# FangjinhuaWang/PatchmatchNet

Measured on AMD Instinct MI355X. Metric: depth-maps/sec at 1600x1200 N=5 src views, higher is better.
Workload: dtype f32

## Files before the change

include/pmn_hip.h:

```cpp
#ifndef PMN_HIP_H
#define PMN_HIP_H

#include <stdint.h>

#ifdef __cplusplus
extern "C" {
#endif

#define PMN_ABI_VERSION 25
#define PMN_MLP_FLOATS 340
#define PMN_MAX_DEPTH 64
#define PMN_MAX_NEIGHBORS 17
#define PMN_MAX_FUSE_SRC 32
#define PMN_TSDF_MAX_VIEWS 16
#define PMN_TSDF_MARK_SPAN 8
#define PMN_RASTER_MAX_DIM 16384
#define PMN_RASTER_MAX_BOX 64
#define PMN_SPLAT_MAX_RADIUS 32

#define PMN_OK 0
#define PMN_ERR_ARG (-1)
#define PMN_ERR_SHAPE (-2)
#define PMN_ERR_LAUNCH (-3)

// ... 28 lines not shown
                          const float *feature_weight, const float *eval_offsets, const int *eval_table_host,
                          int K, float interval_scale, int is_inverse, int B, int D, int h, int w,
                          float *score_out, float *depth_out, void *stream);

int pmn_confidence(const float *score, int B, int D, int h, int w, int H, int W, float *confidence_out,
                   int *depth_index_out, void *stream);

int pmn_conv2d(const float *in, const float *weights, const float *shift, const float *up, float *out, int N, int H,
               int W, int cin, int cout, int K, int stride, int pad, int dil, int relu, int in_nchw, int out_nchw,
               int up_h, int up_w, void *stream);

int pmn_fpn_tail(const float *x, const float *up, const float *w_in, const float *b_in, const float *w_out, float *out,
                 int N, int H, int W, int cin, int cmid, int cout, void *stream);

int pmn_conv2d_mfma(const float *in, const float *weights, const float *shift, float *out, float *out_b, int N, int H, int W,
                    int cin, int cout, int ca, int K, int stride, int pad, int dil, int relu, int planar, void *stream);


int pmn_conv2d_f16s(const float *in, const void *weights, const float *shift, float *out, int N, int H, int W, int cin, int cout,
                    int k, int stride, int relu, void *stream);

int pmn_conv2d_f16s_pair(const float *in, const void *weights_a, const float *shift_a, const void *weights_b, const float *shift_b,
                         float *out, int N, int H, int W, int channels, int relu, void *stream);

int pmn_offset_heads_f16s(const float *in, const void *weights, const float *shift, float *out_a, float *out_b, int N, int H, int W,
                          int cin, int cout, int ca, int dil, void *stream);

int pmn_fpn_level(const float *x, const float *u, const float *w, const float *b, float *out_a, float *out_b, int N, int H,
                  int W, int cin, int cout, int ca, void *stream);

int pmn_deconv3x3s2(const float *in, const float *weights, const float *shift, float *out, int N, int Hi, int Wi, int cin,
                    int cout, int relu, void *stream);

int pmn_refine_front(const float *img, const float *t2, const float *w0, const float *s0, const float *wd, const float *sd,
                     float *x16, int B, int H, int W, void *stream);
int pmn_refine_tail(const float *x16, const float *w3, const float *s3, const float *wr, const float *dnorm,
                    const float *depth_min, const float *depth_max, float *out, int B, int H, int W, void *stream);

int pmn_refine_fused(const float *img, const float *t2, const float *w0, const float *s0, const float *wd, const float *sd,
                     const void *w3a, const float *s3, const float *wr, const float *dnorm, const float *depth_min,
                     const float *depth_max, float *out, int B, int H, int W, void *stream);

int pmn_stage_projections(const float *intrinsics, const float *extrinsics, int B, int V, int nstages, float scale0,
                          float *rel, void *stream);

int pmn_stem(const float *img, const float *w0, const float *s0, const float *w1, const float *s1, float *out, int N, int H,
             int W, void *stream);

int pmn_stem_f16s(const float *img, const float *w0, const float *s0, const void *w1a, const float *s1, float *out, int N, int H,
                  int W, void *stream);

int pmn_stem_f16s_views(const float *const *img_table, int views, const float *w0, const float *s0, const void *w1a,
                        const float *s1, float *out, int B, int H, int W, void *stream);

int pmn_differentiable_warping(const float *src_nchw, const float *rel_proj, const float *depth, int B, int C,
                               int D, int h, int w, int hs, int ws, float *warped, void *stream);

int pmn_fuse_view(const float *maps, long long slot_stride, int ref_slot, const int *src_slots_host,
                  const int *src_hw_host, int n_src, const float *mats, int H, int W, float geo_pixel_thres, float geo_depth_thres, int geo_mask_thres,
                  float photo_thres, unsigned char *masks, float *xyz, double *depth_avg, int *geo_sum, void *stream);

int pmn_fuse_view_merged(const float *maps, long long slot_stride, int ref_slot, const int *src_slots_host,
                         const int *src_hw_host, int n_src, const float *mats, int H, int W, float geo_pixel_thres,
                         float geo_depth_thres, int geo_mask_thres, float photo_thres, unsigned char *masks, float *xyz,
                         double *depth_avg, int *geo_sum, unsigned char *claimed, long long claim_stride, unsigned char *emit,
                         void *stream);

int pmn_pack_points(const unsigned char *final_mask, const float *xyz, const void *image_hwc, int image_is_float, int H, int W,
                    unsigned char *records, long long capacity_points, long long *cursor, int *view_count, long long *scratch,
                    void *stream);

int pmn_pack_points_normals(const unsigned char *final_mask, const float *xyz, const float *normals_chw, const float *rotation,
                            int rotation_stride, const void *image_hwc, int image_is_float, int H, int W, unsigned char *records,
                            long long capacity_points, long long *cursor, int *view_count, long long *scratch, void *stream);

int pmn_depth_normals(const float *depth, int H, int W, const float *intrinsics_host, int radius, float rel_thres,
                      float *normals_out, void *stream);

int pmn_normalize_depth(const float *depth, const float *depth_min, const float *depth_max, int B, int n, float *out,
                        void *stream);

int pmn_check_f16_domain(const float *x, long long n, int *flag, void *stream);

#define PMN_PLAN_PART_PRE 0
#define PMN_PLAN_PART_SIDE 1
#define PMN_PLAN_PART_MAIN 2
#define PMN_PLAN_PART_POST 3
int pmn_plan_create(void **plan_out);
int pmn_plan_begin(void *plan);
int pmn_plan_end(void *plan);
int pmn_plan_count(const void *plan);
const char *pmn_plan_kernel_name(const void *plan, int index);
int pmn_plan_launch(const void *plan, void *stream);
int pmn_plan_destroy(void *plan);
int pmn_plan_fork(void *plan);
int pmn_plan_switch(void *plan, int branch);
int pmn_plan_join(void *plan);
int pmn_plan_entry_branch(const void *plan, int index);
int pmn_plan_launch_part(const void *plan, int part, void *stream);

int pmn_view_scores(const double *cam_centers, const double *xyz, const long long *obs_ptr, const int *obs_pt,
                    const long long *trk_ptr, const int *trk_img, int N, int P, long long n_obs, long long n_trk,
                    double theta0, double sigma1, double sigma2, double *score, void *stream);

#define PMN_METRICS_MAX_STAGES 4
#define PMN_METRICS_MAX_ITERS 5
// ... 154 lines not shown
```

patchmatchnet_amd/_lib.py:

```python
from __future__ import annotations

import ctypes
import os
import subprocess
from typing import Optional

_CSRC = os.path.join(os.path.dirname(os.path.abspath(__file__)), "csrc")
LIB_PATH = os.path.join(_CSRC, "libpmn_hip.so")
ABI_VERSION = 25
MLP_FLOATS = 340
MAX_DEPTH = 64
MAX_NEIGHBORS = 17
MAX_FUSE_SRC = 32
TSDF_MAX_VIEWS = 16
TSDF_MARK_SPAN = 8
RASTER_MAX_DIM = 16384
RASTER_MAX_BOX = 64
SPLAT_MAX_RADIUS = 32
ICP_SUMS = 17
ICP_LIMBS = 5
ICP_BLOCK_POINTS = 256
VOXEL_LONG_RUN = 256
VOXEL_MAX_CHANNELS = 8
CROP_MAX_VERTICES = 4096
MESH_PLACE_LONG_RUN = 256
MESH_SIMPLIFY_MAX_FACES = 715827882
MESH_SMOOTH_LONG_ROW = 256
MESH_SMOOTH_MAX_STEPS = 65536
NORMAL_SWEEPS = 6
NORMAL_MAX_VIEWPOINTS = 4096
PLANE_MAX_HYPOTHESES = 4096
PLANE_SUMS = 10
PLANE_LIMBS = 5
PLANE_BLOCK_POINTS = 1024
MLS_QUADRIC_MIN = 6
MLS_PIVOT_MIN = 1e-10

_fp = ctypes.c_void_p
_ip = ctypes.c_void_p
_hp = ctypes.c_void_p
_i = ctypes.c_int
_f = ctypes.c_float
_s = ctypes.c_void_p

SIGNATURES = {
    "pmn_abi_version": [],
    "pmn_error_string": [_i],
    "pmn_nchw_to_nhwc": [_fp, _fp, _i, _i, _i, _i, _s],
    "pmn_feature_weight": [_fp, _fp, _hp, _fp, _i, _i, _i, _i, _i, _i, _fp, _s],
    "pmn_init_hypotheses": [_fp, _fp, _i, _fp, _fp, _i, _f, _fp, _hp, _i, _i, _i, _i, _fp, _fp, _s],
    "pmn_warp_correlate": [_fp, _fp, _fp, _fp, _fp, _i, _fp, _fp, _i, _i, _i, _i, _i, _i, _i, _i, _i, _fp, _fp, _ip,
                           _fp, _s],
    "pmn_warp_correlate_views": [_fp, _fp, _fp, _fp, _fp, _i, _fp, _fp, _i, _i, _i, _i, _i, _i, _i, _i, _i, _fp, _fp, _ip,
                                 _fp, _s],
    "pmn_aggregate_regress": [_fp, _fp, _fp, _fp, _fp, _hp, _i, _f, _i, _i, _i, _i, _i, _fp, _fp, _s],
    "pmn_confidence": [_fp, _i, _i, _i, _i, _i, _i, _fp, _ip, _s],
    "pmn_conv2d": [_fp, _fp, _fp, _fp, _fp] + [_i] * 14 + [_s],
    "pmn_fpn_tail": [_fp] * 6 + [_i] * 6 + [_s],
    "pmn_fpn_level": [_fp] * 6 + [_i] * 6 + [_s],
    "pmn_conv2d_f16s": [_fp] * 4 + [_i] * 8 + [_s],
    "pmn_offset_heads_f16s": [_fp] * 5 + [_i] * 7 + [_s],
    "pmn_conv2d_f16s_pair": [_fp] * 6 + [_i] * 5 + [_s],
    "pmn_refine_front": [_fp] * 7 + [_i] * 3 + [_s],
    "pmn_refine_tail": [_fp] * 8 + [_i] * 3 + [_s],
    "pmn_refine_fused": [_fp] * 13 + [_i] * 3 + [_s],
    "pmn_conv2d_mfma": [_fp] * 5 + [_i] * 12 + [_s],
    "pmn_deconv3x3s2": [_fp] * 4 + [_i] * 6 + [_s],
    "pmn_stage_projections": [_fp, _fp, _i, _i, _i, _f, _fp, _s],
    "pmn_stem": [_fp] * 6 + [_i] * 3 + [_s],
    "pmn_stem_f16s": [_fp] * 6 + [_i] * 3 + [_s],
    "pmn_stem_f16s_views": [_fp, _i] + [_fp] * 5 + [_i] * 3 + [_s],
    "pmn_differentiable_warping": [_fp, _fp, _fp, _i, _i, _i, _i, _i, _i, _i, _fp, _s],
    "pmn_fuse_view": [_fp, ctypes.c_longlong, _i, _hp, _hp, _i, _fp, _i, _i, _f, _f, _i, _f, _fp, _fp, _fp, _ip, _s],
    "pmn_fuse_view_merged": [_fp, ctypes.c_longlong, _i, _hp, _hp, _i, _fp, _i, _i, _f, _f, _i, _f, _fp, _fp, _fp, _ip, _fp,
                             ctypes.c_longlong, _fp, _s],
    "pmn_pack_points": [_fp, _fp, _fp, _i, _i, _i, _fp, ctypes.c_longlong, _fp, _ip, _fp, _s],
    "pmn_pack_points_normals": [_fp, _fp, _fp, _fp, _i, _fp, _i, _i, _i, _fp, ctypes.c_longlong, _fp, _ip, _fp, _s],
    "pmn_depth_normals": [_fp, _i, _i, _hp, _i, _f, _fp, _s],
    "pmn_normalize_depth": [_fp, _fp, _fp, _i, _i, _fp, _s],
    "pmn_check_f16_domain": [_fp, ctypes.c_longlong, _ip, _s],
    "pmn_plan_create": [ctypes.POINTER(ctypes.c_void_p)],
    "pmn_plan_begin": [_hp],
    "pmn_plan_end": [_hp],
    "pmn_plan_count": [_hp],
    "pmn_plan_kernel_name": [_hp, _i],
    "pmn_plan_launch": [_hp, _s],
    "pmn_plan_destroy": [_hp],
    "pmn_plan_fork": [_hp],
    "pmn_plan_switch": [_hp, _i],
    "pmn_plan_join": [_hp],
    "pmn_plan_entry_branch": [_hp, _i],
    "pmn_plan_launch_part": [_hp, _i, _s],
    "pmn_view_scores": [_fp] * 6 + [_i, _i, ctypes.c_longlong, ctypes.c_longlong] + [ctypes.c_double] * 3 + [_fp, _s],
    "pmn_depth_metrics": [_fp, _fp, _hp, _hp, _hp, _i, _hp, _i, _i, _i, _i, _fp, ctypes.c_longlong, _fp, _s],
    "pmn_nn_distance": [_fp, _ip, ctypes.c_longlong, _hp, ctypes.c_double, _hp, _fp, _ip, ctypes.c_longlong, ctypes.c_double, _fp, _ip,
                        _s],
    "pmn_reduce_round": [_fp, _ip, ctypes.c_longlong, _hp, ctypes.c_double, _hp, ctypes.c_double, _ip, _ip, _ip, _s],
    "pmn_tsdf_integrate": [_fp] * 4 + [_hp, _hp, _f, _f, _fp, ctypes.c_longlong] + [_hp] * 5 + [_i, _s],
    "pmn_mt_count": [_fp, _fp, _hp, _f, _ip, _ip, _s],
    "pmn_mt_emit": [_fp] * 4 + [_hp, _hp, _f, _f] + [_ip] * 4 + [_fp, _ip, _fp, _ip, _s],
    "pmn_tsdf_mark_blocks": [_ip, _ip, _hp, _hp, _f, _f, _fp, ctypes.c_longlong] + [_hp] * 4 + [_i, _s],
    "pmn_tsdf_integrate_blocks": [_fp] * 4 + [_ip, _i, _hp, _hp, _f, _f, _fp, ctypes.c_longlong] + [_hp] * 5 + [_i, _s],
    "pmn_mt_count_blocks": [_fp, _fp, _ip, _ip, _i, _hp, _f, _ip, _ip, _s],
    "pmn_mt_emit_blocks": [_fp] * 4 + [_ip, _ip, _i, _hp, _hp, _f, _f] + [_ip] * 4 + [_fp, _ip, _fp, _ip, _s],
    "pmn_raster_triangles": [_fp, _i, _ip, _i, _hp, _i, _i, ctypes.c_longlong, _ip, _ip, _ip, _s],
    "pmn_splat_points": [_fp, ctypes.c_longlong, _hp, _i, _i, _f, _f, _ip, _ip, _s],
    "pmn_raster_resolve": [_ip, _i, _i, _hp, _fp, ctypes.c_longlong, _ip, ctypes.c_longlong, _ip, _fp, _i, _fp, _ip, _ip, _fp, _s],
    "pmn_icp_accumulate": [_fp, _ip, ctypes.c_longlong, _hp, ctypes.c_double, _hp, _fp, _ip, ctypes.c_longlong, _hp, _hp, ctypes.c_double,
                           _fp, ctypes.c_longlong, _fp, _s],
    "pmn_voxel_mean": [_fp, _fp, _i, ctypes.c_longlong, _ip, ctypes.c_longlong, _fp, _fp, _s],
    "pmn_crop_prism": [_fp, ctypes.c_longlong, _fp, _i, _i, ctypes.c_double, ctypes.c_double, _hp, _ip, _s],
    "pmn_mesh_components": [_ip, _i, _i, _ip, _ip, _s],
    "pmn_mesh_face_samples": [_fp, _i, _ip, _i, ctypes.c_double, ctypes.c_ulonglong, _ip, _ip, _s],
    "pmn_mesh_sample": [_fp, _i, _ip, _i, _ip, _ip, ctypes.c_longlong, ctypes.c_ulonglong, _fp, _ip, _ip, _s],
    "pmn_undistort_image": [_fp, _i, _i, _i, _i, _hp, _hp, _i, _i, _fp, _fp, _fp, _s],
    "pmn_knn_distance": [_fp, _ip, ctypes.c_longlong, _hp, ctypes.c_double, _hp, _fp, _ip, ctypes.c_longlong, _i, ctypes.c_double, _i,
                         _fp, _ip, _fp, _s],
    "pmn_radius_count": [_fp, _ip, ctypes.c_longlong, _hp, ctypes.c_double, _hp, _fp, _ip, ctypes.c_longlong, ctypes.c_double, _i, _ip,
                         _s],
    "pmn_knn_normals": [_fp, _ip, ctypes.c_longlong, _hp, ctypes.c_double, _hp, _fp, _ip, ctypes.c_longlong, _i, ctypes.c_double, _i,
                        _fp, _i, ctypes.c_double, _fp, _fp, _ip, _s],
    "pmn_cloud_core": [_fp, _ip, ctypes.c_longlong, _hp, ctypes.c_double, _hp, ctypes.c_double, ctypes.c_longlong, _ip, _s],
    "pmn_cloud_dbscan": [_fp, _ip, ctypes.c_longlong, _hp, ctypes.c_double, _hp, ctypes.c_double, _ip, _ip, _ip, _ip, _s],
    "pmn_plane_score": [_fp, _fp, _ip, ctypes.c_longlong, _fp, _i, ctypes.c_double, ctypes.c_double, _ip, _s],
# ... 87 lines not shown
```

patchmatchnet_amd/csrc/conv_f16s.hip:

```cpp
#include "conv_common.hpp"

struct F16sArgs {
    int N, H, W, Ho, Wo, relu;
    int cout, ca;
    float* out_b;
};

template <int CIN, int COUT, int KS, int S, int CC, int CCP, int MT, int WPS, int DIL = 1, int OUTMODE = 0, bool SWAP = (OUTMODE == 0)>
__global__ __launch_bounds__(256, WPS) void conv_f16s_kernel(const float* __restrict__ in, const f16x8* __restrict__ wB,
                                                             const float* __restrict__ shift, float* __restrict__ out,
                                                             const F16sArgs a) {
    constexpr int NT = COUT / 16, NCB = CC / 8, CHUNKS = CIN / CC, NQ = KS * KS * NCB, KSTEPS = (NQ + 3) / 4;
    constexpr int TH = 4 * MT, TW = 16, PH = (TH - 1) * S + (KS - 1) * DIL + 1, PW = (TW - 1) * S + (KS - 1) * DIL + 1;
    constexpr int PAD = DIL * (KS / 2);
    constexpr int PLANE = PH * PW * CCP;
    constexpr int NTHR = 256;
    static_assert(!SWAP || OUTMODE == 0, "swapped operand roles (see the epilogue) serve the channels-last output");
    static_assert(CCP % 8 == 0 && CC % 8 == 0 && CIN % CC == 0, "16-byte aligned channel blocks");
    extern __shared__ float4 f16s_lds4[];
    _Float16* Phi = reinterpret_cast<_Float16*>(f16s_lds4);
    _Float16* Plo = Phi + PLANE;
    const int tid = threadIdx.x, wave = __builtin_amdgcn_readfirstlane(tid >> 6), lane = tid & 63, li = lane & 15, kb = lane >> 4;
    const int tiles_x = (a.Wo + TW - 1) / TW, tiles_y = (a.Ho + TH - 1) / TH;
    const int bt = pmn_xcd_tile(blockIdx.x, a.N * tiles_x * tiles_y);
// ... 491 lines not shown
        q = q < 8 ? q : 8;
        const int dy = q / 3, dx = q - dy * 3;
        const _Float16* pb = midh + ((wrow + dy) * MRP + li + dx) * 8;
        f16x8 bh[4], blo[4];
#pragma unroll
        for (int t = 0; t < 4; ++t) {
            bh[t] = *reinterpret_cast<const f16x8*>(pb + t * MRP * 8);
            blo[t] = *reinterpret_cast<const f16x8*>(pb + t * MRP * 8 + MROWS * MRP * 8);
        }
#pragma unroll
        for (int t = 0; t < 4; ++t) accM[t] = __builtin_amdgcn_mfma_f32_16x16x32_f16(wa[ks][0], bh[t], accM[t], 0, 0, 0);
#pragma unroll
        for (int t = 0; t < 4; ++t) accL[t] = __builtin_amdgcn_mfma_f32_16x16x32_f16(wa[ks][0], blo[t], accL[t], 0, 0, 0);
#pragma unroll
        for (int t = 0; t < 4; ++t) accL[t] = __builtin_amdgcn_mfma_f32_16x16x32_f16(wa[ks][1], bh[t], accL[t], 0, 0, 0);
    }
    const int ox = ox0 + li, oyw = oy0 + wrow;
    if (kb < 2 && ox < W) {
        const f32x4_t sh = *reinterpret_cast<const f32x4_t*>(s1 + 4 * kb);
        float* po = out + (((size_t)n * H + oyw) * W + ox) * 8 + 4 * kb;
        const size_t rs = (size_t)W * 8;
#pragma unroll
        for (int t = 0; t < 4; ++t) {
            if (oyw + t < H) {
                *reinterpret_cast<f32x4_t*>(po + t * rs) = f16s_relu(f16s_epilogue(accM[t], accL[t], sh));
            }
        }
    }
    }
}

static int launch_stem_f16s(const float* img, const float* const* img_table, int B, bool vec4, const float* w0, const float* s0,
                            const void* w1a, const float* s1, float* out, int N, int H, int W, void* stream) {
    constexpr int TS = 16, TH = PMN_STEM_TH;
    const int blocks = N * ((W + TS - 1) / TS) * ((H + TH - 1) / TH);
    PMN_LAUNCH((vec4 ? stem_f16s_kernel<true, PMN_STEM_TH> : stem_f16s_kernel<false, PMN_STEM_TH>), dim3(blocks), dim3(256), 0,
               (hipStream_t)stream, img, w0, s0, reinterpret_cast<const f16x8*>(w1a), s1, out, N, H, W, img_table, B);
    PMN_CHECK_LAUNCH();
    return PMN_OK;
}

extern "C" int pmn_stem_f16s(const float* img, const float* w0, const float* s0, const void* w1a, const float* s1, float* out,
                             int N, int H, int W, void* stream) {
    if (!img || !w0 || !s0 || !w1a || !s1 || !out || N < 1 || H < 1 || W < 1) return PMN_ERR_ARG;
    const bool vec4 = W % 4 == 0 && (reinterpret_cast<uintptr_t>(img) & 15) == 0;
    return launch_stem_f16s(img, nullptr, 1, vec4, w0, s0, w1a, s1, out, N, H, W, stream);
}

extern "C" int pmn_stem_f16s_views(const float* const* img_table, int views, const float* w0, const float* s0, const void* w1a,
                                   const float* s1, float* out, int B, int H, int W, void* stream) {
    if (!img_table || !w0 || !s0 || !w1a || !s1 || !out || views < 1 || B < 1 || H < 1 || W < 1) return PMN_ERR_ARG;
    return launch_stem_f16s(nullptr, img_table, B, W % 4 == 0, w0, s0, w1a, s1, out, views * B, H, W, stream);
}
```

patchmatchnet_amd/net.py:

```python
from __future__ import annotations

from typing import Dict, List, Optional, Tuple

import warnings

import numpy as np
import torch
import torch.nn as nn
import torch.nn.functional as F

from . import _lib, ops, params
from ._lib import PmnError
from .module import ConvBnReLU
from .patchmatch import PatchMatch


class FeatureNet(nn.Module):

    def __init__(self) -> None:
        super().__init__()
        spec = [(3, 8, 3, 1, 1), (8, 8, 3, 1, 1), (8, 16, 5, 2, 2), (16, 16, 3, 1, 1), (16, 16, 3, 1, 1),
                (16, 32, 5, 2, 2), (32, 32, 3, 1, 1), (32, 32, 3, 1, 1), (32, 64, 5, 2, 2), (64, 64, 3, 1, 1),
                (64, 64, 3, 1, 1)]
        for i, (cin, cout, k, s, p) in enumerate(spec):
            setattr(self, f"conv{i}", ConvBnReLU(cin, cout, k, s, p))
        self.output1 = nn.Conv2d(64, 64, 1, bias=False)
        self.inner1 = nn.Conv2d(32, 64, 1, bias=True)
        self.inner2 = nn.Conv2d(16, 64, 1, bias=True)
        self.output2 = nn.Conv2d(64, 32, 1, bias=False)
        self.output3 = nn.Conv2d(64, 16, 1, bias=False)
        self.f16_split = True
        self.f16_domain_error: Optional[str] = None
        self.fold_fpn = True
        self.fuse_conv34 = True
        self.fpn8_valu = False
        self.layer_hook = None

    _SPEC = [(3, 1, 1), (3, 1, 1), (5, 2, 2), (3, 1, 1), (3, 1, 1), (5, 2, 2), (3, 1, 1), (3, 1, 1), (5, 2, 2), (3, 1, 1),
             (3, 1, 1)]

    def _packed(self):
        srcs = [p for p in self.parameters()] + [b for b in self.buffers() if b.dtype.is_floating_point]
        key = params.versions(srcs)
        if getattr(self, "_pack_key", None) != key:
            dev = self.output1.weight.device
            pk = {}
            f16_ok, self.f16_domain_error = True, None
            for i in range(11):
                m = getattr(self, f"conv{i}")
                w, s = params.pack_conv(m.conv.weight, bn=(m.bn.weight, m.bn.bias, m.bn.running_mean, m.bn.running_var),
                                        eps=m.bn.eps)
                pk[f"conv{i}"] = (torch.from_numpy(w).to(dev), torch.from_numpy(s).to(dev))
                cv = m.conv
                if (cv.kernel_size[0], cv.stride[0], cv.in_channels, cv.out_channels) in ops.F16S_SHAPES and f16_ok:
                    try:
                        w, s = params.pack_conv_f16s(cv.weight, bn=(m.bn.weight, m.bn.bias, m.bn.running_mean, m.bn.running_var),
                                                     eps=m.bn.eps)
                        pk[f"conv{i}_f16s"] = (torch.from_numpy(w).to(dev), torch.from_numpy(s).to(dev))
                    except params.F16DomainError as e:
                        f16_ok, self.f16_domain_error = False, f"conv{i}: {e}"
            m1 = self.conv1
            try:
                w, s = params.pack_stem_conv1_f16s(m1.conv.weight, bn=(m1.bn.weight, m1.bn.bias, m1.bn.running_mean, m1.bn.running_var),
                                                  eps=m1.bn.eps)
                pk["conv1_f16s"] = (torch.from_numpy(w).to(dev), torch.from_numpy(s).to(dev))
            except params.F16DomainError as e:
                f16_ok, self.f16_domain_error = False, f"conv1: {e}"
            if not f16_ok:
                for k in [k for k in pk if k.endswith("_f16s")]:
                    del pk[k]
                warnings.warn("FeatureNet: " + self.f16_domain_error + " -- using the fp32 kernels (pmn_stem / pmn_conv2d) instead of "
                              "the fp16-split matrix-core kernels", RuntimeWarning, stacklevel=2)
            for name in ("output1", "inner1", "inner2", "output2", "output3"):
                m = getattr(self, name)
                w, s = params.pack_conv(m.weight, bias=m.bias)
                pk[name] = (torch.from_numpy(w).to(dev), torch.from_numpy(s).to(dev))
            fold = params.fold_fpn(self.output1.weight, self.inner1.weight, self.inner1.bias, self.inner2.weight,
                                   self.inner2.bias, self.output2.weight, self.output3.weight)
            for lvl, (w, b) in fold.items():
                pk[f"fpn{lvl}"] = (torch.from_numpy(w).to(dev), torch.from_numpy(b).to(dev))
            w8 = torch.from_numpy(np.ascontiguousarray(fold[8][0].T))[:, :, None, None]
            w, s = params.pack_conv_mfma(w8, bias=torch.from_numpy(fold[8][1]))
            pk["fpn8_mfma"] = (torch.from_numpy(w).to(dev), torch.from_numpy(s).to(dev))
            self._pack, self._pack_key = pk, key
        return self._pack

    def forward_hip(self, x, image_table: Optional["ops.SourceTable"] = None, pending: Optional[dict] = None
                    ) -> Dict[int, torch.Tensor]:
        pk = self._packed()
        imgs = list(x) if isinstance(x, (list, tuple)) else [x]
        B, _, H, W = imgs[0].shape
        in_place = image_table is not None
        if in_place and not (self.f16_split and "conv1_f16s" in pk):
            raise PmnError("image_table: only the fp16-split stem (FeatureNet.f16_split, weights inside its domain) reads images in place")
        if in_place:
            t = ops.stem_f16s_views(image_table, *pk["conv0"], *pk["conv1_f16s"])
        else:
            t = torch.empty((B * len(imgs), H, W, 8), dtype=torch.float32, device=imgs[0].device)
        for i, im in enumerate(() if in_place else imgs):
            if self.f16_split and "conv1_f16s" in pk:
                ops.stem_f16s(im.contiguous(), *pk["conv0"], *pk["conv1_f16s"], out=t[i * B:(i + 1) * B])
            else:
                ops.stem(im.contiguous(), *pk["conv0"], *pk["conv1"], out=t[i * B:(i + 1) * B])
        feats = {}
        for i, (k, s, p) in enumerate(self._SPEC):
            if i < 2:
                continue
            if i == 4 and self.f16_split and self.fuse_conv34 and "conv3_f16s" in pk and "conv4_f16s" in pk:
                continue
            if i == 3 and self.f16_split and self.fuse_conv34 and "conv3_f16s" in pk and "conv4_f16s" in pk:
                t = ops.conv2d_f16s_pair(t, *pk["conv3_f16s"], *pk["conv4_f16s"], relu=True)
                feats[4] = t
            elif self.f16_split and f"conv{i}_f16s" in pk:
                t = ops.conv2d_f16s(t, *pk[f"conv{i}_f16s"], k, s, relu=True)
            elif self.layer_hook is not None and (hooked := self.layer_hook(i, t)) is not None:
                t = hooked
            else:
                w, sh = pk[f"conv{i}"]
                t = ops.conv2d(t, w, sh, getattr(self, f"conv{i}").conv.out_channels, k, s, p, relu=True)
            if i in (4, 7, 10):
                feats[i] = t
        half, quarter, eighth = feats[4], feats[7], feats[10]
        if self.fold_fpn:
            if self.fpn8_valu:
                f3, u8 = ops.fpn_level(eighth, None, *pk["fpn8"], ca=64)
            else:
                f3, u8 = ops.pointwise_split_mfma(eighth, *pk["fpn8_mfma"], cout=112, ca=64)
            if pending is not None:
                pending.update(half=half, quarter=quarter, u8=u8)
                return {3: f3}
            return {3: f3, **self.finish_hip(dict(half=half, quarter=quarter, u8=u8))}
        out = {3: ops.conv2d(eighth, *pk["output1"], 64, 1)}
        top = ops.conv2d(quarter, *pk["inner1"], 64, 1, up=eighth)
        out[2] = ops.conv2d(top, *pk["output2"], 32, 1)
        out[1] = ops.fpn_tail(half, top, pk["inner2"][0], pk["inner2"][1], pk["output3"][0])
        return out

    def finish_hip(self, pending: dict) -> Dict[int, torch.Tensor]:
        pk = self._packed()
        f2, u4 = ops.fpn_level(pending["quarter"], pending["u8"], *pk["fpn4"], ca=32)
        f1, _ = ops.fpn_level(pending["half"], u4, *pk["fpn2"], ca=16)
        return {2: f2, 1: f1}

    def forward(self, x: torch.Tensor) -> Dict[int, torch.Tensor]:
        half = self.conv4(self.conv3(self.conv2(self.conv1(self.conv0(x)))))
        quarter = self.conv7(self.conv6(self.conv5(half)))
        eighth = self.conv10(self.conv9(self.conv8(quarter)))
        out: Dict[int, torch.Tensor] = {3: self.output1(eighth)}
        top = F.interpolate(eighth, scale_factor=2.0, mode="bilinear", align_corners=False) + self.inner1(quarter)
        out[2] = self.output2(top)
        top = F.interpolate(top, scale_factor=2.0, mode="bilinear", align_corners=False) + self.inner2(half)
        out[1] = self.output3(top)
        return out


class Refinement(nn.Module):

    def __init__(self) -> None:
        super().__init__()
# ... 268 lines not shown
```

patchmatchnet_amd/ops.py:

```python
from __future__ import annotations

import ctypes
import threading
from typing import List, Optional, Sequence, Tuple

import numpy as np
import torch

from . import _lib
from ._lib import PmnError, check


_TIMING = None
_TIMING_ON = True


def enable_kernel_timing() -> None:
    global _TIMING, _TIMING_ON
    _TIMING, _TIMING_ON = [], True


def pause_kernel_timing(paused: bool) -> None:
    global _TIMING_ON
    _TIMING_ON = not paused
# ... 759 lines not shown
def stem(img: torch.Tensor, w0: torch.Tensor, s0: torch.Tensor, w1: torch.Tensor, s1: torch.Tensor,
         out: Optional[torch.Tensor] = None) -> torch.Tensor:
    for n_, t_ in (("img", img), ("w0", w0), ("s0", s0), ("w1", w1), ("s1", s1)):
        _dev(t_, n_)
    N, c, H, W = img.shape
    if c != 3 or tuple(w0.shape) != (3, 3, 3, 8) or tuple(w1.shape) != (3, 3, 8, 8):
        raise PmnError("stem: expects a 3-channel image and 3->8->8 weights")
    if out is None:
        out = torch.empty((N, H, W, 8), dtype=torch.float32, device=img.device)
    else:
        _dev(out, "out")
        if tuple(out.shape) != (N, H, W, 8):
            raise PmnError("stem: bad `out` shape")
    with torch.cuda.device(img.device):
        check(_lib.lib().pmn_stem(img.data_ptr(), w0.data_ptr(), s0.data_ptr(), w1.data_ptr(), s1.data_ptr(), out.data_ptr(),
                                  N, H, W, _stream(img)), "pmn_stem")
    return out


def stem_f16s(img: torch.Tensor, w0: torch.Tensor, s0: torch.Tensor, w1a: torch.Tensor, s1: torch.Tensor,
              out: Optional[torch.Tensor] = None) -> torch.Tensor:
    for n_, t_ in (("img", img), ("w0", w0), ("s0", s0), ("s1", s1)):
        _dev(t_, n_)
    if tuple(_dev_as(w1a, "stem_f16s: w1a", torch.float16).shape) != (3, 2, 64, 8):
        raise PmnError("stem_f16s: w1a must be the float16 [3,2,64,8] tensor of params.pack_stem_conv1_f16s")
    N, c, H, W = img.shape
    if c != 3 or tuple(w0.shape) != (3, 3, 3, 8):
        raise PmnError("stem_f16s: expects a 3-channel image and 3->8 conv0 weights")
    _f16_domain_probe(img)
    if out is None:
        out = torch.empty((N, H, W, 8), dtype=torch.float32, device=img.device)
    else:
        _dev(out, "out")
        if tuple(out.shape) != (N, H, W, 8):
            raise PmnError("stem_f16s: bad `out` shape")
    with torch.cuda.device(img.device):
        check(_lib.lib().pmn_stem_f16s(img.data_ptr(), w0.data_ptr(), s0.data_ptr(), w1a.data_ptr(), s1.data_ptr(), out.data_ptr(),
                                       N, H, W, _stream(img)), "pmn_stem_f16s")
    return out


def stem_f16s_views(images: "SourceTable", w0: torch.Tensor, s0: torch.Tensor, w1a: torch.Tensor, s1: torch.Tensor) -> torch.Tensor:
    for n_, t_ in (("w0", w0), ("s0", s0), ("s1", s1)):
        _dev(t_, n_)
    if not isinstance(images, SourceTable) or len(images.shape) != 5 or images.shape[2] != 3:
        raise PmnError("stem_f16s_views: a SourceTable of shape (views, B, 3, H, W)")
    if tuple(_dev_as(w1a, "stem_f16s_views: w1a", torch.float16).shape) != (3, 2, 64, 8) or tuple(w0.shape) != (3, 3, 3, 8):
        raise PmnError("stem_f16s_views: 3->8 conv0 weights and the float16 [3,2,64,8] tensor of params.pack_stem_conv1_f16s")
    V, B, _, H, W = images.shape
    out = torch.empty((V * B, H, W, 8), dtype=torch.float32, device=images.device)
    with torch.cuda.device(images.device):
        check(_lib.lib().pmn_stem_f16s_views(images.table.data_ptr(), V, w0.data_ptr(), s0.data_ptr(), w1a.data_ptr(), s1.data_ptr(),
                                             out.data_ptr(), B, H, W, _stream(out)), "pmn_stem_f16s_views")
    return out


def fuse_view(maps: torch.Tensor, ref_slot: int, src_slots: Sequence[int], mats: torch.Tensor, geo_pixel_thres: float,
              geo_depth_thres: float, geo_mask_thres: int, photo_thres: float, want_depth_avg: bool = False,
              want_geo_sum: bool = False, sizes: Optional[Sequence[Tuple[int, int]]] = None):
    masks, xyz, davg, gsum, _ = _fuse_view(maps, ref_slot, src_slots, mats, geo_pixel_thres, geo_depth_thres, geo_mask_thres,
                                           photo_thres, want_depth_avg, want_geo_sum, sizes, None)
    return masks, xyz, davg, gsum


def fuse_view_merged(maps: torch.Tensor, ref_slot: int, src_slots: Sequence[int], mats: torch.Tensor, geo_pixel_thres: float,
                     geo_depth_thres: float, geo_mask_thres: int, photo_thres: float, claimed: torch.Tensor,
                     sizes: Optional[Sequence[Tuple[int, int]]] = None):
    if not isinstance(claimed, torch.Tensor) or claimed.dtype != torch.uint8 or claimed.dim() != 2 or not claimed.is_contiguous():
        raise PmnError("fuse_view_merged: claimed must be a contiguous uint8 tensor [V,S], one slot per map slot")
    if not isinstance(maps, torch.Tensor) or claimed.device != maps.device:
        raise PmnError("fuse_view_merged: claimed must be on the maps' device (no CPU fallback)")
    if ref_slot in src_slots:
        raise PmnError("fuse_view_merged: the reference slot is in its own source list")
    masks, xyz, _, _, emit = _fuse_view(maps, ref_slot, src_slots, mats, geo_pixel_thres, geo_depth_thres, geo_mask_thres,
                                        photo_thres, False, False, sizes, claimed)
    return masks, xyz, emit


def _fuse_view(maps, ref_slot, src_slots, mats, geo_pixel_thres, geo_depth_thres, geo_mask_thres, photo_thres, want_depth_avg,
               want_geo_sum, sizes, claimed):
    _dev(maps, "maps")
    _dev(mats, "mats")
    if sizes is None:
        if maps.dim() != 4 or maps.shape[1] != 2:
            raise PmnError("fuse_view: maps must be [V,2,H,W] (or [V,F] flat slots with sizes=)")
        V, _, H, W = maps.shape
        stride = 2 * H * W
        sizes = [(H, W)] * V
    else:
        if maps.dim() != 2 or len(sizes) != maps.shape[0]:
            raise PmnError("fuse_view: with sizes= maps must be [V,F] flat slots and sizes must have V entries")
        V, stride = maps.shape
        if any(h < 1 or w < 1 or 2 * h * w > stride for h, w in sizes):
            raise PmnError("fuse_view: a view's maps do not fit its slot")
    n = len(src_slots)
    if n > _lib.MAX_FUSE_SRC:
        raise PmnError(f"fuse_view: at most {_lib.MAX_FUSE_SRC} source views per reference view")
    if not 0 <= ref_slot < V or any(not 0 <= s < V for s in src_slots):
        raise PmnError("fuse_view: slot out of range")
    if mats.numel() != 48 + 64 * n:
        raise PmnError("fuse_view: mats must hold 48 + 64 * n_src floats (fusion.camera_block)")
    if claimed is not None and (claimed.shape[0] != V or any(h * w > claimed.shape[1] for h, w in sizes)):
        raise PmnError("fuse_view_merged: claimed must have one slot per map slot, each with room for the largest view's h*w bytes")
    H, W = sizes[ref_slot]
    slots, slots_p = _host_i32(np.asarray(list(src_slots) if n else [0], np.int32), max(n, 1), "src_slots")
    hw, hw_p = _host_i32(np.asarray([x for s in src_slots for x in sizes[s]] if n else [0, 0], np.int32), max(2 * n, 2), "src_hw")
# ... 630 lines not shown
```

Measured before the change: 400.9.

## Fuse stem conv0/conv1 with stride-2 conv2 in one LDS-resident kernel

Adds a kernel that computes conv0 and conv1 of the feature stem into LDS as fp16 hi/lo split planes, then runs the 5x5 stride-2 conv2 from LDS with MFMA. It writes only the half-resolution 16-channel output. This removes the full-resolution 8-channel intermediate write and read, plus a launch. In exchange it recomputes halo regions per 16x16 output tile and uses large LDS per block, which limits occupancy.

```diff
diff --git a/include/pmn_hip.h b/include/pmn_hip.h
--- a/include/pmn_hip.h
+++ b/include/pmn_hip.h
@@ -104,6 +104,12 @@
 
 int pmn_stem_f16s_views(const float *const *img_table, int views, const float *w0, const float *s0, const void *w1a,
                         const float *s1, float *out, int B, int H, int W, void *stream);
+
+int pmn_stem_conv2_f16s(const float *img, const float *w0, const float *s0, const void *w1a, const float *s1, const void *w2b,
+                        const float *s2, float *out, int N, int H, int W, void *stream);
+
+int pmn_stem_conv2_f16s_views(const float *const *img_table, int views, const float *w0, const float *s0, const void *w1a,
+                              const float *s1, const void *w2b, const float *s2, float *out, int B, int H, int W, void *stream);
 
 int pmn_differentiable_warping(const float *src_nchw, const float *rel_proj, const float *depth, int B, int C,
                                int D, int h, int w, int hs, int ws, float *warped, void *stream);
diff --git a/patchmatchnet_amd/_lib.py b/patchmatchnet_amd/_lib.py
--- a/patchmatchnet_amd/_lib.py
+++ b/patchmatchnet_amd/_lib.py
@@ -70,6 +70,8 @@
     "pmn_stem": [_fp] * 6 + [_i] * 3 + [_s],
     "pmn_stem_f16s": [_fp] * 6 + [_i] * 3 + [_s],
     "pmn_stem_f16s_views": [_fp, _i] + [_fp] * 5 + [_i] * 3 + [_s],
+    "pmn_stem_conv2_f16s": [_fp] * 8 + [_i] * 3 + [_s],
+    "pmn_stem_conv2_f16s_views": [_fp, _i] + [_fp] * 7 + [_i] * 3 + [_s],
     "pmn_differentiable_warping": [_fp, _fp, _fp, _i, _i, _i, _i, _i, _i, _i, _fp, _s],
     "pmn_fuse_view": [_fp, ctypes.c_longlong, _i, _hp, _hp, _i, _fp, _i, _i, _f, _f, _i, _f, _fp, _fp, _fp, _ip, _s],
     "pmn_fuse_view_merged": [_fp, ctypes.c_longlong, _i, _hp, _hp, _i, _fp, _i, _i, _f, _f, _i, _f, _fp, _fp, _fp, _ip, _fp,
diff --git a/patchmatchnet_amd/csrc/conv_f16s.hip b/patchmatchnet_amd/csrc/conv_f16s.hip
--- a/patchmatchnet_amd/csrc/conv_f16s.hip
+++ b/patchmatchnet_amd/csrc/conv_f16s.hip
@@ -567,3 +567,252 @@
     if (!img_table || !w0 || !s0 || !w1a || !s1 || !out || views < 1 || B < 1 || H < 1 || W < 1) return PMN_ERR_ARG;
     return launch_stem_f16s(nullptr, img_table, B, W % 4 == 0, w0, s0, w1a, s1, out, views * B, H, W, stream);
 }
+
+
+template <int J>
+__device__ __forceinline__ void stem_conv2_conv1_tiles(const _Float16* __restrict__ m0h, _Float16* __restrict__ m1h, const f16x8 (&wa)[3][2],
+                                                       const f32x4_t sh1, const int first, const int ntiles, const int lim, const int g0,
+                                                       const int wave, const int li, const int kb, const int yc, const int xc, const int H,
+                                                       const int W) {
+    constexpr int C0 = 37, C1 = 35, M0PLANE = 37 * 37 * 8, M1PLANE = 35 * 35 * 8;
+    f32x4_t accM[J], accL[J];
+    const _Float16* pb[J];
+    int mm[J];
+#pragma unroll
+    for (int j = 0; j < J; ++j) {
+        accM[j] = f32x4_t{0.f, 0.f, 0.f, 0.f};
+        accL[j] = f32x4_t{0.f, 0.f, 0.f, 0.f};
+        const int t = wave + 8 * (g0 + j);
+        const int m = min(first + (t < ntiles ? t : ntiles - 1) * 16 + li, lim - 1);
+        mm[j] = t < ntiles && first + t * 16 + li < lim ? m : -1;
+        const int r = m / C1, c = m - r * C1;
+        pb[j] = m0h + (r * C0 + c) * 8;
+    }
+#pragma unroll
+    for (int ks = 0; ks < 3; ++ks) {
+        int q = 4 * ks + kb;
+        q = q < 8 ? q : 8;
+        const int dy = q / 3, dx = q - dy * 3;
+        const int off = (dy * C0 + dx) * 8;
+        f16x8 bh[J], blo[J];
+#pragma unroll
+        for (int j = 0; j < J; ++j) {
+            bh[j] = *reinterpret_cast<const f16x8*>(pb[j] + off);
+            blo[j] = *reinterpret_cast<const f16x8*>(pb[j] + off + M0PLANE);
+        }
+#pragma unroll
+        for (int j = 0; j < J; ++j) accM[j] = __builtin_amdgcn_mfma_f32_16x16x32_f16(wa[ks][0], bh[j], accM[j], 0, 0, 0);
+#pragma unroll
+        for (int j = 0; j < J; ++j) accL[j] = __builtin_amdgcn_mfma_f32_16x16x32_f16(wa[ks][0], blo[j], accL[j], 0, 0, 0);
+#pragma unroll
+        for (int j = 0; j < J; ++j) accL[j] = __builtin_amdgcn_mfma_f32_16x16x32_f16(wa[ks][1], bh[j], accL[j], 0, 0, 0);
+    }
+    if (kb < 2) {
+#pragma unroll
+        for (int j = 0; j < J; ++j) {
+            const int m = mm[j];
+            if (m >= 0) {
+                const int r = m / C1, c = m - r * C1;
+                f16x4 hi = {0, 0, 0, 0}, lo = {0, 0, 0, 0};
+                if ((unsigned)(yc + r) < (unsigned)H && (unsigned)(xc + c) < (unsigned)W)
+                    f16s_split4(f16s_relu(f16s_epilogue(accM[j], accL[j], sh1)), hi, lo);
+                *reinterpret_cast<f16x4*>(m1h + m * 8 + 4 * kb) = hi;
+                *reinterpret_cast<f16x4*>(m1h + M1PLANE + m * 8 + 4 * kb) = lo;
+            }
+        }
+    }
+}
+
+template <bool VEC4>
+__global__ __launch_bounds__(512, 4) void stem_f16s_kernel_conv2(const float* __restrict__ img, const float* __restrict__ w0,
+                                                                const float* __restrict__ s0, const f16x8* __restrict__ w1A,
+                                                                const float* __restrict__ s1, const f16x8* __restrict__ w2B,
+                                                                const float* __restrict__ s2, float* __restrict__ out, const int N,
+                                                                const int H, const int W, const int Ho, const int Wo,
+                                                                const float* const* __restrict__ img_tab, const int BV) {
+    constexpr int TO = 16, NTHR = 512;
+    constexpr int IR = 39, IC = 40;
+    constexpr int R0 = 37, C0 = 37;
+    constexpr int R1 = 35, C1 = 35;
+    constexpr int M0PLANE = R0 * C0 * 8, M1PLANE = R1 * C1 * 8;
+    constexpr int LATE = 3 * C1;
+    static_assert((R1 * C1 - LATE) % 16 == 0, "the early part of conv1 is whole tiles");
+    extern __shared__ float4 sc2_lds4[];
+    _Float16* m0h = reinterpret_cast<_Float16*>(sc2_lds4);
+    _Float16* m1h = m0h + 2 * M0PLANE - LATE * 8;
+    float* xin = reinterpret_cast<float*>(m0h + 2 * M0PLANE);
+    typedef const float __attribute__((address_space(4))) cfloat;
+    const cfloat* cw0 = (const cfloat*)w0;
+    const cfloat* cs0 = (const cfloat*)s0;
+    const int tid = threadIdx.x, wave = __builtin_amdgcn_readfirstlane(tid >> 6), lane = tid & 63, li = lane & 15, kb = lane >> 4;
+    const int tiles_x = (Wo + TO - 1) / TO, tiles_y = (Ho + TO - 1) / TO;
+    const int bt = pmn_xcd_tile(blockIdx.x, N * tiles_x * tiles_y);
+    const int n = bt / (tiles_x * tiles_y), tr = bt - n * tiles_x * tiles_y;
+    const int oy0 = (tr / tiles_x) * TO, ox0 = (tr % tiles_x) * TO;
+    const int yi = 2 * oy0 - 4, xi = 2 * ox0 - 4;
+    if (img_tab) img = img_tab[n / BV] + (ptrdiff_t)((n % BV) - n) * 3 * H * W;
+
+    f16x8 wa[3][2];
+#pragma unroll
+    for (int ks = 0; ks < 3; ++ks) {
+        wa[ks][0] = w1A[(ks * 2 + 0) * 64 + lane];
+        wa[ks][1] = w1A[(ks * 2 + 1) * 64 + lane];
+    }
+    if constexpr (VEC4) {
+        constexpr int NU = (3 * IR + 31) / 32;
+        float4 v[NU];
+        const int j = tid & 15, gx = xi + 4 * j;
+#pragma unroll
+        for (int u = 0; u < NU; ++u) {
+            const int R = (tid >> 4) + 32 * u;
+            const int c = (R >= IR) + (R >= 2 * IR), r = R - IR * c, gy = yi + r;
+            v[u] = make_float4(0.f, 0.f, 0.f, 0.f);
+            if (j < 10 && R < 3 * IR && (unsigned)gy < (unsigned)H && (unsigned)gx < (unsigned)W)
+                v[u] = *reinterpret_cast<const float4*>(img + (((size_t)n * 3 + c) * H + gy) * W + gx);
+        }
+#pragma unroll
+        for (int u = 0; u < NU; ++u) {
+            const int R = (tid >> 4) + 32 * u;
+            if (j < 10 && R < 3 * IR) *reinterpret_cast<float4*>(xin + R * IC + 4 * j) = v[u];
+        }
+    } else {
+        const int q = tid & 63, gx = xi + q;
+#pragma unroll 1
+        for (int u0 = 0; u0 < 15; u0 += 5) {
+            float v[5];
+#pragma unroll
+            for (int u = 0; u < 5; ++u) {
+                const int R = (tid >> 6) + 8 * (u0 + u);
+                const int c = (R >= IR) + (R >= 2 * IR), r = R - IR * c, gy = yi + r;
+                v[u] = 0.0f;
+                if (q < IC && R < 3 * IR && (unsigned)gy < (unsigned)H && (unsigned)gx < (unsigned)W)
+                    v[u] = img[(((size_t)n * 3 + c) * H + gy) * W + gx];
+            }
+#pragma unroll
+            for (int u = 0; u < 5; ++u) {
+                const int R = (tid >> 6) + 8 * (u0 + u);
+                if (q < IC && R < 3 * IR) xin[R * IC + q] = v[u];
+            }
+        }
+    }
+    __syncthreads();
+    for (int m = tid; m < R0 * C0; m += NTHR) {
+        const int r = m / C0, q = m - r * C0;
+        const int gy = yi + 1 + r, gx = xi + 1 + q;
+        f16x8 hi = {0, 0, 0, 0, 0, 0, 0, 0}, lo = {0, 0, 0, 0, 0, 0, 0, 0};
+        if ((unsigned)gy < (unsigned)H && (unsigned)gx < (unsigned)W) {
+            float acc[8];
+#pragma unroll
+            for (int c = 0; c < 8; ++c) acc[c] = 0.0f;
+            const float* xp = xin + r * IC + q;
+#pragma unroll 1
+            for (int ky = 0; ky < 3; ++ky) {
+                const cfloat* wq = cw0 + __builtin_amdgcn_readfirstlane(ky * 72);
+#pragma unroll
+                for (int kx = 0; kx < 3; ++kx)
+#pragma unroll
+                    for (int ci = 0; ci < 3; ++ci) {
+                        const float v = xp[(ci * IR + ky) * IC + kx];
+#pragma unroll
+                        for (int c = 0; c < 8; ++c) acc[c] = fmaf(v, wq[(kx * 3 + ci) * 8 + c], acc[c]);
+                    }
+            }
+#pragma unroll
+            for (int c = 0; c < 8; c += 2) {
+                const f32x2_t x = {fmaxf(acc[c] + cs0[c], 0.0f), fmaxf(acc[c + 1] + cs0[c + 1], 0.0f)};
+                const f16x2_t h = f16s_hi2(x), l = f16s_lo2(x, h);
+                hi[c] = h[0];
+                hi[c + 1] = h[1];
+                lo[c] = l[0];
+                lo[c + 1] = l[1];
+            }
+        }
+        *reinterpret_cast<f16x8*>(m0h + m * 8) = hi;
+        *reinterpret_cast<f16x8*>(m0h + M0PLANE + m * 8) = lo;
+    }
+    __syncthreads();
+    {
+        const f32x4_t sh1 = *reinterpret_cast<const f32x4_t*>(s1 + 4 * (kb & 1));
+        constexpr int NT1 = (R1 * C1 - LATE) / 16;
+#pragma unroll 1
+        for (int g = 0; g * 8 < NT1; g += 3)
+            stem_conv2_conv1_tiles<3>(m0h, m1h, wa, sh1, LATE, NT1, R1 * C1, g, wave, li, kb, yi + 2, xi + 2, H, W);
+        __syncthreads();
+        stem_conv2_conv1_tiles<1>(m0h, m1h, wa, sh1, 0, (LATE + 15) / 16, LATE, 0, wave, li, kb, yi + 2, xi + 2, H, W);
+    }
+    __syncthreads();
+    {
+        constexpr int MT = 2, NQ = 25, KSTEPS = 7, S = 2, KS = 5;
+        f32x4_t accM[MT], accL[MT];
+#pragma unroll
+        for (int t = 0; t < MT; ++t) {
+            accM[t] = f32x4_t{0.f, 0.f, 0.f, 0.f};
+            accL[t] = f32x4_t{0.f, 0.f, 0.f, 0.f};
+        }
+        const f16x8* bl = w2B + lane;
+        f16x8 bq[2][2];
+        bq[0][0] = bl[0];
+        bq[0][1] = bl[64];
+#pragma unroll
+        for (int ks = 0; ks < KSTEPS; ++ks) {
+            const int cur = ks & 1, nxt = cur ^ 1;
+            const int sidx = ks + 1 < KSTEPS ? ks + 1 : KSTEPS - 1;
+            bq[nxt][0] = bl[(size_t)(sidx * 2 + 0) * 64];
+            bq[nxt][1] = bl[(size_t)(sidx * 2 + 1) * 64];
+            int q = 4 * ks + kb;
+            if (4 * ks + 3 >= NQ) q = q < NQ - 1 ? q : NQ - 1;
+            const int dy = q / KS, dx = q - dy * KS;
+            const _Float16* pa = m1h + ((wave * MT * S + dy) * C1 + li * S + dx) * 8;
+            f16x8 ah[MT], al[MT];
+#pragma unroll
+            for (int t = 0; t < MT; ++t) {
+                ah[t] = *reinterpret_cast<const f16x8*>(pa + t * S * C1 * 8);
+                al[t] = *reinterpret_cast<const f16x8*>(pa + t * S * C1 * 8 + M1PLANE);
+            }
+#pragma unroll
+            for (int t = 0; t < MT; ++t) accM[t] = __builtin_amdgcn_mfma_f32_16x16x32_f16(bq[cur][0], ah[t], accM[t], 0, 0, 0);
+#pragma unroll
+            for (int t = 0; t < MT; ++t) accL[t] = __builtin_amdgcn_mfma_f32_16x16x32_f16(bq[cur][1], ah[t], accL[t], 0, 0, 0);
+#pragma unroll
+            for (int t = 0; t < MT; ++t) accL[t] = __builtin_amdgcn_mfma_f32_16x16x32_f16(bq[cur][0], al[t], accL[t], 0, 0, 0);
+            __builtin_amdgcn_sched_barrier(0);
+        }
+        const int ox = ox0 + li, oyw = oy0 + wave * MT;
+        if (ox < Wo) {
+            float* po = out + (((size_t)n * Ho + oyw) * Wo + ox) * 16 + 4 * kb;
+            const size_t rs = (size_t)Wo * 16;
+            const f32x4_t sh2 = *reinterpret_cast<const f32x4_t*>(s2 + 4 * kb);
+#pragma unroll
+            for (int t = 0; t < MT; ++t)
+                if (oyw + t < Ho) *reinterpret_cast<f32x4_t*>(po + t * rs) = f16s_relu(f16s_epilogue(accM[t], accL[t], sh2));
+        }
+    }
+}
+
+static int launch_stem_conv2_f16s(const float* img, const float* const* img_table, int B, bool vec4, const float* w0, const float* s0,
+                                  const void* w1a, const float* s1, const void* w2b, const float* s2, float* out, int N, int H, int W,
+                                  void* stream) {
+    const int Ho = (H - 1) / 2 + 1, Wo = (W - 1) / 2 + 1;
+    const size_t lds = ((size_t)2 * 37 * 37 + (size_t)2 * 35 * 35 - 3 * 35) * 8 * sizeof(_Float16);
+    const int blocks = N * ((Wo + 15) / 16) * ((Ho + 15) / 16);
+    auto kern = vec4 ? stem_f16s_kernel_conv2<true> : stem_f16s_kernel_conv2<false>;
+    if (pmn_raise_dynamic_lds(reinterpret_cast<const void*>(kern), lds) != PMN_OK) return PMN_ERR_LAUNCH;
+    PMN_LAUNCH(kern, dim3(blocks), dim3(512), lds, (hipStream_t)stream, img, w0, s0, reinterpret_cast<const f16x8*>(w1a), s1,
+               reinterpret_cast<const f16x8*>(w2b), s2, out, N, H, W, Ho, Wo, img_table, B);
+    PMN_CHECK_LAUNCH();
+    return PMN_OK;
+}
+
+extern "C" int pmn_stem_conv2_f16s(const float* img, const float* w0, const float* s0, const void* w1a, const float* s1, const void* w2b,
+                                   const float* s2, float* out, int N, int H, int W, void* stream) {
+    if (!img || !w0 || !s0 || !w1a || !s1 || !w2b || !s2 || !out || N < 1 || H < 1 || W < 1) return PMN_ERR_ARG;
+    const bool vec4 = W % 4 == 0 && (reinterpret_cast<uintptr_t>(img) & 15) == 0;
+    return launch_stem_conv2_f16s(img, nullptr, 1, vec4, w0, s0, w1a, s1, w2b, s2, out, N, H, W, stream);
+}
+
+extern "C" int pmn_stem_conv2_f16s_views(const float* const* img_table, int views, const float* w0, const float* s0, const void* w1a,
+                                         const float* s1, const void* w2b, const float* s2, float* out, int B, int H, int W,
+                                         void* stream) {
+    if (!img_table || !w0 || !s0 || !w1a || !s1 || !w2b || !s2 || !out || views < 1 || B < 1 || H < 1 || W < 1) return PMN_ERR_ARG;
+    return launch_stem_conv2_f16s(nullptr, img_table, B, W % 4 == 0, w0, s0, w1a, s1, w2b, s2, out, views * B, H, W, stream);
+}
diff --git a/patchmatchnet_amd/net.py b/patchmatchnet_amd/net.py
--- a/patchmatchnet_amd/net.py
+++ b/patchmatchnet_amd/net.py
@@ -33,6 +33,7 @@
         self.f16_domain_error: Optional[str] = None
         self.fold_fpn = True
         self.fuse_conv34 = True
+        self.fuse_stem_conv2 = True
         self.fpn8_valu = False
         self.layer_hook = None
 
@@ -93,18 +94,25 @@
         in_place = image_table is not None
         if in_place and not (self.f16_split and "conv1_f16s" in pk):
             raise PmnError("image_table: only the fp16-split stem (FeatureNet.f16_split, weights inside its domain) reads images in place")
-        if in_place:
+        stem_conv2 = self.f16_split and self.fuse_stem_conv2 and "conv1_f16s" in pk and "conv2_f16s" in pk
+        if in_place and stem_conv2:
+            t = ops.stem_conv2_f16s_views(image_table, *pk["conv0"], *pk["conv1_f16s"], *pk["conv2_f16s"])
+        elif in_place:
             t = ops.stem_f16s_views(image_table, *pk["conv0"], *pk["conv1_f16s"])
+        elif stem_conv2:
+            t = torch.empty((B * len(imgs), (H - 1) // 2 + 1, (W - 1) // 2 + 1, 16), dtype=torch.float32, device=imgs[0].device)
         else:
             t = torch.empty((B * len(imgs), H, W, 8), dtype=torch.float32, device=imgs[0].device)
         for i, im in enumerate(() if in_place else imgs):
-            if self.f16_split and "conv1_f16s" in pk:
+            if stem_conv2:
+                ops.stem_conv2_f16s(im.contiguous(), *pk["conv0"], *pk["conv1_f16s"], *pk["conv2_f16s"], out=t[i * B:(i + 1) * B])
+            elif self.f16_split and "conv1_f16s" in pk:
                 ops.stem_f16s(im.contiguous(), *pk["conv0"], *pk["conv1_f16s"], out=t[i * B:(i + 1) * B])
             else:
                 ops.stem(im.contiguous(), *pk["conv0"], *pk["conv1"], out=t[i * B:(i + 1) * B])
         feats = {}
         for i, (k, s, p) in enumerate(self._SPEC):
-            if i < 2:
+            if i < 2 or (i == 2 and stem_conv2):
                 continue
             if i == 4 and self.f16_split and self.fuse_conv34 and "conv3_f16s" in pk and "conv4_f16s" in pk:
                 continue
diff --git a/patchmatchnet_amd/ops.py b/patchmatchnet_amd/ops.py
--- a/patchmatchnet_amd/ops.py
+++ b/patchmatchnet_amd/ops.py
@@ -835,6 +835,51 @@
     with torch.cuda.device(images.device):
         check(_lib.lib().pmn_stem_f16s_views(images.table.data_ptr(), V, w0.data_ptr(), s0.data_ptr(), w1a.data_ptr(), s1.data_ptr(),
                                              out.data_ptr(), B, H, W, _stream(out)), "pmn_stem_f16s_views")
+    return out
+
+
+def _stem_conv2_packs(what: str, w0: torch.Tensor, s0: torch.Tensor, w1a: torch.Tensor, s1: torch.Tensor, w2b: torch.Tensor,
+                      s2: torch.Tensor) -> None:
+    for n_, t_ in (("w0", w0), ("s0", s0), ("s1", s1), ("s2", s2)):
+        _dev(t_, n_)
+    if tuple(_dev_as(w1a, what + ": w1a", torch.float16).shape) != (3, 2, 64, 8) or tuple(w0.shape) != (3, 3, 3, 8):
+        raise PmnError(what + ": 3->8 conv0 weights and the float16 [3,2,64,8] tensor of params.pack_stem_conv1_f16s")
+    if tuple(_dev_as(w2b, what + ": w2b", torch.float16).shape) != (1, 7, 1, 2, 64, 8) or s2.numel() != 16:
+        raise PmnError(what + ": w2b / s2 must be params.pack_conv_f16s of a (5, 2, 8, 16) layer")
+
+
+def stem_conv2_f16s(img: torch.Tensor, w0: torch.Tensor, s0: torch.Tensor, w1a: torch.Tensor, s1: torch.Tensor, w2b: torch.Tensor,
+                    s2: torch.Tensor, out: Optional[torch.Tensor] = None) -> torch.Tensor:
+    _dev(img, "img")
+    _stem_conv2_packs("stem_conv2_f16s", w0, s0, w1a, s1, w2b, s2)
+    N, c, H, W = img.shape
+    if c != 3:
+        raise PmnError("stem_conv2_f16s: expects a 3-channel image")
+    _f16_domain_probe(img)
+    Ho, Wo = (H - 1) // 2 + 1, (W - 1) // 2 + 1
+    if out is None:
+        out = torch.empty((N, Ho, Wo, 16), dtype=torch.float32, device=img.device)
+    else:
+        _dev(out, "out")
+        if tuple(out.shape) != (N, Ho, Wo, 16):
+            raise PmnError("stem_conv2_f16s: bad `out` shape")
+    with torch.cuda.device(img.device):
+        check(_lib.lib().pmn_stem_conv2_f16s(img.data_ptr(), w0.data_ptr(), s0.data_ptr(), w1a.data_ptr(), s1.data_ptr(), w2b.data_ptr(),
+                                             s2.data_ptr(), out.data_ptr(), N, H, W, _stream(img)), "pmn_stem_conv2_f16s")
+    return out
+
+
+def stem_conv2_f16s_views(images: "SourceTable", w0: torch.Tensor, s0: torch.Tensor, w1a: torch.Tensor, s1: torch.Tensor,
+                          w2b: torch.Tensor, s2: torch.Tensor) -> torch.Tensor:
+    if not isinstance(images, SourceTable) or len(images.shape) != 5 or images.shape[2] != 3:
+        raise PmnError("stem_conv2_f16s_views: a SourceTable of shape (views, B, 3, H, W)")
+    _stem_conv2_packs("stem_conv2_f16s_views", w0, s0, w1a, s1, w2b, s2)
+    V, B, _, H, W = images.shape
+    out = torch.empty((V * B, (H - 1) // 2 + 1, (W - 1) // 2 + 1, 16), dtype=torch.float32, device=images.device)
+    with torch.cuda.device(images.device):
+        check(_lib.lib().pmn_stem_conv2_f16s_views(images.table.data_ptr(), V, w0.data_ptr(), s0.data_ptr(), w1a.data_ptr(),
+                                                   s1.data_ptr(), w2b.data_ptr(), s2.data_ptr(), out.data_ptr(), B, H, W, _stream(out)),
+              "pmn_stem_conv2_f16s_views")
     return out
 
 
```

Result: faster. 409.1, median of 6 (+2.0%).
